# YuhuaXu/ImageMosaicing

Measured on AMD Instinct MI355X. Metric: image-pairs/sec (detect+match+H+warp), 4000x3000 UAV frames, higher is better.
Workload: dtype i16 fixed-point pyramid filtered in f32 (as the reference's OpenCV), f32 (RANSAC / warp coordinates), int8 MFMA with int32 accumulation (descriptor distances, exact), u8 (pixels); 1 GPU; C3: ONE 500-frame 4000x3000 UAV survey, pair window 2 (499 pairs), SIFT(2000,3,0.01,20) + exact BF match + 3x3 grid select + Ransac2D + MosaicImagesRefined warp; frames=500, pairs=499, frames_per_gpu=500, pairs_per_gpu=499

## Files before the change

imagemosaicing_amd/csrc/sift.hip:

```cpp
#include "common.h"
#include <memory>
#include "detmath.h"
#include <cmath>
#include <type_traits>

namespace {

constexpr int N_LAYERS = 3, N_LEVELS = 6, IMG_BORDER = 5, MAX_INTERP = 5, ORI_BINS = 36, MAX_OCT = 16;
constexpr int FIXPT_SCALE = 48;
constexpr float DOG_THRESHOLD_P1 = 21.0f;
constexpr float HIST_Q = 1024.0f;
constexpr int MAX_R = 16;
constexpr int SIFT_BATCH_MAX = MI355_SIFT_BATCH_MAX;
typedef int16_t lvl_t;

__host__ __device__ __forceinline__ int reflect101(int p, int n) {
    if (n == 1) return 0;
    while (p < 0 || p >= n) { if (p < 0) p = -p; else p = 2 * n - 2 - p; }
    return p;
}

typedef float v2f __attribute__((ext_vector_type(2)));
struct __attribute__((aligned(4))) uint2_a4 { unsigned x, y; };
typedef float v4f __attribute__((ext_vector_type(4)));

__device__ __forceinline__ v4f ld4(const lvl_t* p) {
    const uint2 q = *reinterpret_cast<const uint2*>(p);
    v4f o;
    o.x = (float)(int)(short)(q.x & 0xffffu); o.y = (float)((int)q.x >> 16);
    o.z = (float)(int)(short)(q.y & 0xffffu); o.w = (float)((int)q.y >> 16);
    return o;
}
__device__ __forceinline__ float ld1(const lvl_t* p) { return (float)(int)*p; }
__device__ __forceinline__ int sat16(float v) {
    int q = (int)rintf(v);
    q = q < -32768 ? -32768 : (q > 32767 ? 32767 : q);
    return q;
}
__device__ __forceinline__ float gray48(const uint8_t* p) {
    return (float)(((1868 * (int)p[0] + 9617 * (int)p[1] + 4899 * (int)p[2] + 8192) >> 14) * FIXPT_SCALE);
}

__device__ __forceinline__ int xcd_remap(int bid, int nb) {
    const int q = nb >> 3, r = nb & 7, xcd = bid & 7, local = bid >> 3;
    const int base = xcd < r ? xcd * (q + 1) : r * (q + 1) + (xcd - r) * q;
    return base + local;
}

template <int J, int NPP, class F> __device__ __forceinline__ bool static_rows(F& f) {
    if constexpr (J < NPP) { if (!f(std::integral_constant<int, J>{})) return false; return static_rows<J + 1, NPP>(f); }
    else return true;
}

struct Blur16Args {
    const lvl_t* src;
    const uint8_t* bgr[SIFT_BATCH_MAX];
    int bgr_ws[SIFT_BATCH_MAX];
    lvl_t* dst;
    lvl_t* ds;
    int w, h;
    int tiles_x, tiles_y;
    float k[2 * MAX_R + 1];
    float kp[2 * (MAX_R + 1)];
    size_t fstride;
    int nb;
};

constexpr int T16W = 64, T16H = 32;
template <int R, bool BGR>
__global__ __launch_bounds__(256) void blur16_tile(Blur16Args a) {
    constexpr int ROWS = T16H + 2 * R, COLS = T16W + 2 * R, PIN = COLS | 1, PMID = T16W + 4;
    __shared__ float s_in[ROWS * PIN];
    __shared__ __attribute__((aligned(16))) float s_mid[ROWS * PMID];
    const int tid = threadIdx.x, fr = blockIdx.y;
    const int tile = xcd_remap(blockIdx.x, a.tiles_x * a.tiles_y);
    const int ty = tile / a.tiles_x, tx = tile - ty * a.tiles_x;
    const int x0 = tx * T16W, y0 = ty * T16H;
    const lvl_t* src = BGR ? nullptr : a.src + (size_t)fr * a.fstride;
    const uint8_t* bgr = a.bgr[0]; int bws = a.bgr_ws[0];
    if (BGR) {
#pragma unroll
        for (int q = 1; q < SIFT_BATCH_MAX; q++) if (fr == q) { bgr = a.bgr[q]; bws = a.bgr_ws[q]; }
    }
    lvl_t* dst = a.dst + (size_t)fr * a.fstride;
    for (int idx = tid; idx < ROWS * COLS; idx += 256) {
        const int ry = idx / COLS, rx = idx - ry * COLS;
        const int gy = reflect101(y0 - R + ry, a.h), gx = reflect101(x0 - R + rx, a.w);
        s_in[ry * PIN + rx] = BGR ? gray48(bgr + (size_t)gy * bws + 3 * gx) : ld1(src + (size_t)gy * a.w + gx);
    }
    __syncthreads();
    for (int item = tid; item < ROWS * (T16W / 4); item += 256) {
        const int xg = item / ROWS, row = item - xg * ROWS;
        const float* in = s_in + row * PIN + 4 * xg;
        float e[2 * R + 4];
#pragma unroll
        for (int m = 0; m < 2 * R + 4; m++) e[m] = in[m];
        float acc[4];
#pragma unroll
        for (int q = 0; q < 4; q++) acc[q] = a.k[0] * e[q];
#pragma unroll
        for (int i = 1; i <= 2 * R; i++) {
#pragma unroll
            for (int q = 0; q < 4; q++) { const float p = a.k[i] * e[q + i]; acc[q] = acc[q] + p; }
        }
        *reinterpret_cast<v4f*>(s_mid + row * PMID + 4 * xg) = (v4f){acc[0], acc[1], acc[2], acc[3]};
    }
    __syncthreads();
    for (int item = tid; item < T16H * (T16W / 4); item += 256) {
        const int yy = item / (T16W / 4), xg = item - yy * (T16W / 4);
        const float* mid = s_mid + (yy + R) * PMID + 4 * xg;
        v4f acc = *reinterpret_cast<const v4f*>(mid) * a.k[R];
#pragma unroll
        for (int j = 1; j <= R; j++) {
            const v4f sm = *reinterpret_cast<const v4f*>(mid + j * PMID) + *reinterpret_cast<const v4f*>(mid - j * PMID);
            const v4f p = sm * a.k[R + j];
            acc = acc + p;
        }
        const int gx = x0 + 4 * xg, gy = y0 + yy;
        if (gy >= a.h) continue;
        const int o0 = sat16(acc.x), o1 = sat16(acc.y), o2 = sat16(acc.z), o3 = sat16(acc.w);
        lvl_t* d = dst + (size_t)gy * a.w + gx;
        if (gx + 3 < a.w && (a.w & 3) == 0) {
            *reinterpret_cast<uint2*>(d) = make_uint2((unsigned)(o0 & 0xffff) | ((unsigned)o1 << 16), (unsigned)(o2 & 0xffff) | ((unsigned)o3 << 16));
        } else {
            if (gx < a.w) d[0] = (lvl_t)o0;
            if (gx + 1 < a.w) d[1] = (lvl_t)o1;
            if (gx + 2 < a.w) d[2] = (lvl_t)o2;
            if (gx + 3 < a.w) d[3] = (lvl_t)o3;
        }
        if (a.ds && !(gy & 1) && (gy >> 1) < (a.h >> 1)) {
            lvl_t* q = a.ds + (size_t)fr * a.fstride + (size_t)(gy >> 1) * (a.w >> 1);
            if ((gx >> 1) < (a.w >> 1)) q[gx >> 1] = (lvl_t)o0;
            if (((gx + 2) >> 1) < (a.w >> 1)) q[(gx + 2) >> 1] = (lvl_t)o2;
        }
    }
}

#include "build/blur16_asm.inc"
template <int R, bool BGR, bool DS>
__device__ __forceinline__ void blur16_stream_body(const Blur16Args& a, int L, int nstrip, int nseg) {
    constexpr int RA = (R + 3) / 4 * 4, SW = 256, BW = SW + 2 * RA;
    constexpr int BUF = (BW + 8 + 63) & ~63;
    static_assert(2 * RA + R <= 64, "halo lanes");
    __shared__ __attribute__((aligned(16))) float s_buf[4][2][BUF];
    const int lane = threadIdx.x & 63, wave = threadIdx.x >> 6;
    int unit = __builtin_amdgcn_readfirstlane(xcd_remap(blockIdx.x, gridDim.x) * 4 + wave);
    const int per = nstrip * nseg, fr = unit / per;
    if (fr >= a.nb) return;
    unit -= fr * per;
    const int seg = unit / nstrip, strip = unit - seg * nstrip;
    if (seg >= nseg) return;
    const int x0 = strip * SW, y0 = seg * L;
    const int lact = (a.h - y0 < L) ? a.h - y0 : L;
    const int wv = a.w - x0;
    const int xm = x0 + 4 * lane;
    const int xl = xm < a.w - 4 ? xm : a.w - 4;
    int hcol, hpos;
    if (lane < RA) { hcol = x0 - RA + lane; hpos = lane; }
    else if (lane < 2 * RA) { hcol = x0 + SW + (lane - RA); hpos = SW + lane; }
    else if (wv < SW && lane < 2 * RA + R) { hcol = x0 + wv + (lane - 2 * RA); hpos = RA + wv + (lane - 2 * RA); }
    else { hcol = x0; hpos = BW + (lane & 7); }
    hcol = reflect101(hcol, a.w);
    const size_t fro = (size_t)fr * a.fstride;
    const uint8_t* bgr = a.bgr[0]; int bws = a.bgr_ws[0];
    if (BGR) {
#pragma unroll
        for (int q = 1; q < SIFT_BATCH_MAX; q++) if (fr == q) { bgr = a.bgr[q]; bws = a.bgr_ws[q]; }
    }
    const int rowb = BGR ? bws : 2 * a.w;
    int gy = y0 - R, dir = 1;
    if (gy < 0) { gy = -gy; dir = -1; }
    const unsigned long long rp = (unsigned long long)(BGR ? reinterpret_cast<uintptr_t>(bgr) : reinterpret_cast<uintptr_t>(a.src + fro)) + (unsigned long long)gy * (unsigned)rowb;
    const unsigned moff = BGR ? 3u * xl : 2u * xl;
    unsigned hoff, hsh = 0;
    if (BGR) {
        const int b0 = 3 * hcol; int st = b0 & ~3; if (st + 8 > bws) st = bws - 8;
        hoff = (unsigned)st; hsh = 8u * (unsigned)(b0 - st);
    } else hoff = 2u * hcol;
    const unsigned lds0 = (unsigned)reinterpret_cast<uintptr_t>(&s_buf[wave][0][0]);
    const unsigned lds_win = lds0 + 16u * lane, lds_main = lds0 + 4u * (RA + 4 * lane), lds_halo = lds0 + 4u * hpos;
    const unsigned long long dp = (unsigned long long)reinterpret_cast<uintptr_t>(a.dst + fro) + 2ull * (unsigned long long)y0 * a.w;
    const unsigned long long dsp = DS ? (unsigned long long)reinterpret_cast<uintptr_t>(a.ds + fro) + 2ull * (unsigned long long)(y0 >> 1) * (a.w >> 1) : 0ull;
    const unsigned doff = 2u * xm, dsoff = 2u * (xm >> 1);
    const unsigned long long smask = __ballot(xm < a.w);
    const unsigned long long kp = (unsigned long long)reinterpret_cast<uintptr_t>(__builtin_amdgcn_kernarg_segment_ptr()) + offsetof(Blur16Args, kp);
    const int n = lact + 2 * R + 1;
    const int hm1 = a.h - 1, dstr = 2 * a.w;
    (void)hsh;
#define BLUR_ASM_CALL(NAME) NAME(lds_win, lds_main, lds_halo, moff, hoff, doff, dsoff, rp, dp, dsp, kp, smask, rowb, gy, dir, hm1, dstr, n)
    if constexpr (BGR) { static_assert(R == 6, "base level"); blur16_asm_r6_bgr(lds_win, lds_main, lds_halo, moff, hoff, doff, dsoff, hsh, rp, dp, dsp, kp, smask, rowb, gy, dir, hm1, dstr, n); }
    else if constexpr (R == 5) BLUR_ASM_CALL(blur16_asm_r5);
    else if constexpr (R == 6) BLUR_ASM_CALL(blur16_asm_r6);
    else if constexpr (R == 8 && DS) BLUR_ASM_CALL(blur16_asm_r8_ds);
    else if constexpr (R == 8) BLUR_ASM_CALL(blur16_asm_r8);
    else if constexpr (R == 10) BLUR_ASM_CALL(blur16_asm_r10);
    else if constexpr (R == 13) BLUR_ASM_CALL(blur16_asm_r13);
#undef BLUR_ASM_CALL
}
template <int R, bool BGR, bool DS, int W>
__global__ __launch_bounds__(256) __attribute__((amdgpu_waves_per_eu(W, W))) void blur16_stream(Blur16Args a, int L, int nstrip, int nseg) {
    blur16_stream_body<R, BGR, DS>(a, L, nstrip, nseg);
}

__global__ __launch_bounds__(256) void downsample16(const lvl_t* src, int sw, lvl_t* dst, int dw, int dh, size_t fstride) {
    src += (size_t)blockIdx.z * fstride; dst += (size_t)blockIdx.z * fstride;
    const int x = blockIdx.x * 64 + (threadIdx.x & 63), y = blockIdx.y * 4 + (threadIdx.x >> 6);
    if (x < dw && y < dh) dst[(size_t)y * dw + x] = src[(size_t)(2 * y) * sw + 2 * x];
}

struct OctaveDev { lvl_t* lv[N_LEVELS]; int w, h; };

#ifndef EXT_EH
#define EXT_EH 16
#endif
constexpr int EW = 64, EH = EXT_EH, ECAP = 128;
#ifndef REG_SHIFT_V
#define REG_SHIFT_V 0
#endif
constexpr int REG_SHIFT = REG_SHIFT_V;
constexpr int NREG = 64, REG_STRIDE = 32;
struct BatchStride { size_t pyr, claimed, cand, refined, kps, cube, sel, mins; };
constexpr size_t CNT_STRIDE = 64, CCNT_STRIDE = (size_t)64 * 32, SEL_STRIDE = 2048;
struct FrameOuts { mi355_keypoint* kp[SIFT_BATCH_MAX]; uint8_t* d8[SIFT_BATCH_MAX]; };

struct Refined { int o, layer, r, c; float xi, xr, xc, contr, scl; unsigned start; };

struct PyrDev { OctaveDev oc[MAX_OCT]; unsigned* claimed[MAX_OCT]; unsigned* mins[MAX_OCT]; int n_oct; };

__device__ __forceinline__ float dogv(const OctaveDev& oc, size_t foff, int lvl, int r, int c) {
    const size_t o = foff + (size_t)r * oc.w + c;
    return (float)((int)oc.lv[lvl + 1][o] - (int)oc.lv[lvl][o]);
}

__device__ __forceinline__ void solve3(const float a[3][3], const float b[3], float x[3]) {
    const float det = (a[0][0] * (a[1][1] * a[2][2] - a[2][1] * a[1][2]) - a[0][1] * (a[1][0] * a[2][2] - a[2][0] * a[1][2])) + a[0][2] * (a[1][0] * a[2][1] - a[2][0] * a[1][1]);
    if (det == 0.0f) { x[0] = x[1] = x[2] = 0.0f; return; }
    const float d = 1.0f / det;
    x[0] = d * ((b[0] * (a[1][1] * a[2][2] - a[1][2] * a[2][1]) - a[0][1] * (b[1] * a[2][2] - a[1][2] * b[2])) + a[0][2] * (b[1] * a[2][1] - a[1][1] * b[2]));
    x[1] = d * ((a[0][0] * (b[1] * a[2][2] - a[1][2] * b[2]) - b[0] * (a[1][0] * a[2][2] - a[1][2] * a[2][0])) + a[0][2] * (a[1][0] * b[2] - b[1] * a[2][0]));
    x[2] = d * ((a[0][0] * (a[1][1] * b[2] - b[1] * a[2][1]) - a[0][1] * (a[1][0] * b[2] - b[1] * a[2][0])) + b[0] * (a[1][0] * a[2][1] - a[1][1] * a[2][0]));
}

struct FitOff { float xi, xr, xc; };
template <class DV>
__device__ __forceinline__ FitOff fit_step(DV dv, int L, int R, int C) {
    const float img_scale = 1.0f / (float)(255 * FIXPT_SCALE);
    const float deriv_scale = img_scale * 0.5f, second_scale = img_scale, cross_scale = img_scale * 0.25f;
    float dD[3];
    dD[0] = (dv(L, R, C + 1) - dv(L, R, C - 1)) * deriv_scale;
    dD[1] = (dv(L, R + 1, C) - dv(L, R - 1, C)) * deriv_scale;
    dD[2] = (dv(L + 1, R, C) - dv(L - 1, R, C)) * deriv_scale;
    const float v2 = dv(L, R, C) * 2.0f;
    const float dxx = (dv(L, R, C + 1) + dv(L, R, C - 1) - v2) * second_scale;
    const float dyy = (dv(L, R + 1, C) + dv(L, R - 1, C) - v2) * second_scale;
// ... 220 lines not shown
#pragma unroll
    for (int b = 0; b < 12; b++) out |= ((hit >> (11 - b)) & 1u) << b;
    unsigned cmask = 0;
#pragma unroll
    for (int k = 0; k < 4; k++) cmask |= (xm + k >= clo && xm + k < chi) ? (0x111u << k) : 0u;
    return out & cmask;
}

struct XH { s2 hx[5][2], hn[5][2]; };
struct XCen { s2 v[3][2]; };
__device__ __forceinline__ void xrow_extremes(const XDog& d, XH& h, XCen& c) {
#pragma unroll
    for (int p = 0; p < 5; p++) {
        const unsigned u01 = as_u(d.m[p][0]), u23 = as_u(d.m[p][1]);
        const unsigned l23 = dpp_lower(u23), r01 = dpp_upper(u01);
        const s2 s_m0 = as_s2(__builtin_amdgcn_alignbit(u01, l23, 16));
        const s2 s_12 = as_s2(__builtin_amdgcn_alignbit(u23, u01, 16));
        const s2 s_34 = as_s2(__builtin_amdgcn_alignbit(r01, u23, 16));
        h.hx[p][0] = pmax(pmax(s_m0, d.m[p][0]), s_12); h.hx[p][1] = pmax(pmax(s_12, d.m[p][1]), s_34);
        h.hn[p][0] = pmin(pmin(s_m0, d.m[p][0]), s_12); h.hn[p][1] = pmin(pmin(s_12, d.m[p][1]), s_34);
    }
#pragma unroll
    for (int l = 0; l < 3; l++) { c.v[l][0] = d.m[l + 1][0]; c.v[l][1] = d.m[l + 1][1]; }
}
__device__ __forceinline__ unsigned xtest_rows(const XH& A, const XH& B, const XH& C, const XCen& cen, int xm, int clo, int chi, bool row_ok) {
    s2 hx[5][2], hn[5][2];
#pragma unroll
    for (int p = 0; p < 5; p++)
#pragma unroll
        for (int r = 0; r < 2; r++) { hx[p][r] = pmax(pmax(A.hx[p][r], B.hx[p][r]), C.hx[p][r]); hn[p][r] = pmin(pmin(A.hn[p][r], B.hn[p][r]), C.hn[p][r]); }
    unsigned hit = 0;
    const s2 t21 = {21, 21}, tm21 = {-21, -21};
#pragma unroll
    for (int layer = 1; layer <= N_LAYERS; layer++) {
#pragma unroll
        for (int r = 0; r < 2; r++) {
            const s2 val = cen.v[layer - 1][r];
            const s2 mx = pmax(pmax(pmax(hx[layer - 1][r], hx[layer][r]), hx[layer + 1][r]), t21);
            const s2 mn = pmin(pmin(pmin(hn[layer - 1][r], hn[layer][r]), hn[layer + 1][r]), tm21);
            const bool h0 = (val.x == mx.x) | (val.x == mn.x), h1 = (val.y == mx.y) | (val.y == mn.y);
            hit = (hit << 2) | (h0 ? 2u : 0u) | (h1 ? 1u : 0u);
        }
    }
    if (!row_ok || hit == 0) return 0u;
    unsigned out = 0;
#pragma unroll
    for (int b = 0; b < 12; b++) out |= ((hit >> (11 - b)) & 1u) << b;
    unsigned cmask = 0;
#pragma unroll
    for (int k = 0; k < 4; k++) cmask |= (xm + k >= clo && xm + k < chi) ? (0x111u << k) : 0u;
    return out & cmask;
}

__global__ __launch_bounds__(256) __attribute__((amdgpu_waves_per_eu(XWAVES, XWAVES)))
void extrema_stream(OctaveDev oc, int octave, unsigned long long* cand, unsigned* count, unsigned cap, unsigned* overflow, BatchStride bs,
                    float* cube, unsigned cube_cap, int L, int nstrip, int nseg, int nb, int xsw ) {
    const int lane = threadIdx.x & 63, wave = threadIdx.x >> 6;
    int unit = __builtin_amdgcn_readfirstlane(xcd_remap(blockIdx.x, gridDim.x) * 4 + wave);
    const int per = nstrip * nseg, fr = unit / per;
    if (fr >= nb) return;
    unit -= fr * per;
    {
        const size_t f = (size_t)fr;
#pragma unroll
        for (int l = 0; l < N_LEVELS; l++) oc.lv[l] += f * bs.pyr;
        cand += f * bs.cand; count += f * CCNT_STRIDE; overflow += f * CNT_STRIDE; cube += f * bs.cube;
    }
    const int seg = unit / nstrip, strip = unit - seg * nstrip;
    const int xs = strip * xsw, y0 = seg * L;
    const int lact = (oc.h - y0 < L) ? oc.h - y0 : L;
    const unsigned reg = (unsigned)unit & (NREG - 1);
    const int xm = xs - 4 + 4 * lane;
    const int xl = xm < 0 ? 0 : (xm < oc.w - 4 ? xm : oc.w - 4);
    int clo = xs > IMG_BORDER ? xs : IMG_BORDER, chi = xs + xsw < oc.w - IMG_BORDER ? xs + xsw : oc.w - IMG_BORDER;
    if (lane == 0 || lane == 63) { clo = 0; chi = 0; }
    const int hm1 = oc.h - 1;
    auto load_row = [&](int r, XRow& q) {
        r = r < 0 ? 0 : (r > hm1 ? hm1 : r);
        const size_t o = (size_t)r * oc.w + xl;
#pragma unroll
        for (int l = 0; l < N_LEVELS; l++) q.m[l] = *reinterpret_cast<const uint2*>(oc.lv[l] + o);
    };
    auto to_dog = [&](const XRow& q, XDog& d) {
#pragma unroll
        for (int p = 0; p < 5; p++) { d.m[p][0] = as_s2(q.m[p + 1].x) - as_s2(q.m[p].x); d.m[p][1] = as_s2(q.m[p + 1].y) - as_s2(q.m[p].y); }
    };
    __shared__ unsigned long long s_rec[4][XCAP];
    int nq = 0;
    auto wave_sync = [&]() { __builtin_amdgcn_fence(__ATOMIC_ACQ_REL, "wavefront"); __builtin_amdgcn_wave_barrier(); };
    auto flush = [&]() {
        if (nq == 0) return;
        wave_sync();
        unsigned base = 0;
        if (lane == 0) base = atomicAdd(&count[reg * REG_STRIDE], (unsigned)nq);
        base = __shfl(base, 0);
        for (int idx = lane; idx < nq; idx += 64) {
            const unsigned g = base + (unsigned)idx;
            if (g >= cap) { *overflow = 1; continue; }
            cand[(size_t)reg * cap + g] = s_rec[wave][idx];
        }
        wave_sync();
        nq = 0;
    };
    auto emit = [&](unsigned hit, int rc, auto in_loop) -> bool {
        constexpr bool IN_LOOP = decltype(in_loop)::value;
        const int nq0 = nq;
        while (__builtin_amdgcn_ballot_w64(hit != 0)) {
            const bool mine = hit != 0;
            const int bb = mine ? __builtin_ctz(hit) : 0;
            hit &= hit - 1;
            const unsigned long long m = __builtin_amdgcn_ballot_w64(mine);
// ... 750 lines not shown
        if (q < 2) v = v + (float)(long long)s_hq[idx + n + q] * (1.0f / HIST_Q);
        s_dst[t] = v;
    }
    wave_sync();
    float a = s_dst[lane], b = s_dst[lane + 64];
    auto seq_sum = [&](float va, float vb) {
        const float sa = va * va, sb = vb * vb;
        float acc = 0.0f;
#pragma unroll
        for (int q = 0; q < 64; q++) acc = acc + __int_as_float(__builtin_amdgcn_readlane(__float_as_int(sa), q));
#pragma unroll
        for (int q = 0; q < 64; q++) acc = acc + __int_as_float(__builtin_amdgcn_readlane(__float_as_int(sb), q));
        return acc;
    };
    const float thr = sqrtf(seq_sum(a, b)) * 0.2f;
    a = a < thr ? a : thr; b = b < thr ? b : thr;
    const float nn = sqrtf(seq_sum(a, b));
    const float fac = 512.0f / (nn > 1.1920929e-7f ? nn : 1.1920929e-7f);
    const float va = rintf(a * fac), vb = rintf(b * fac);
    desc[(size_t)kidx * 128 + lane] = (uint8_t)(va < 0.0f ? 0 : (va > 255.0f ? 255 : (int)va));
    desc[(size_t)kidx * 128 + lane + 64] = (uint8_t)(vb < 0.0f ? 0 : (vb > 255.0f ? 255 : (int)vb));
}

int gauss_kernel_host(double sigma, float* k) {
    const int ksize = ((int)lrint(sigma * 8.0 + 1.0)) | 1;
    const int r = ksize / 2;
    double sum = 0.0;
    const double scale2x = -0.5 / (sigma * sigma);
    for (int i = 0; i < ksize; i++) { const double x = (double)i - (double)(ksize - 1) * 0.5; k[i] = (float)std::exp(scale2x * x * x); sum += (double)k[i]; }
    sum = 1.0 / sum;
    for (int i = 0; i < ksize; i++) k[i] = (float)((double)k[i] * sum);
    return r;
}

inline bool blur_streams(const Blur16Args& a, bool bgr, int R, int stream_mode) {
    const bool has_r = bgr ? R == 6 : (R == 5 || R == 6 || R == 8 || R == 10 || R == 13);
    bool ok = stream_mode && has_r && (a.w & 3) == 0 && ((a.w & 255) == 0 || (a.w & 255) > MAX_R) && a.w >= 512 && a.h >= 64;
    if (bgr) { for (int f = 0; f < a.nb; f++) ok = ok && ((uintptr_t)a.bgr[f] & 3) == 0 && (a.bgr_ws[f] & 3) == 0 && a.bgr_ws[f] >= 3 * a.w; }
    else ok = ok && ((uintptr_t)a.src & 7) == 0;
    if (a.ds) ok = ok && R == 8 && (a.h & 1) == 0;
    return ok && ((uintptr_t)a.dst & 7) == 0 && (a.fstride & 3) == 0;
}
inline void stream_grid(int w, int h, int& L, int& nstrip, int& nseg, int nb = 1, int waves = 2) {
    static const int units_env = [] { const char* e = getenv("MI355_STREAM_UNITS"); return e ? atoi(e) : 0; }();
    const int units_target = units_env ? units_env : 1024 * waves;
    static const int stream_minl = [] { const char* e = getenv("MI355_STREAM_MINL"); return e ? atoi(e) : 64; }();
    nstrip = (w + 255) / 256;
    nseg = (units_target + nstrip * nb - 1) / (nstrip * nb);
    L = (h + nseg - 1) / nseg;
    if (L < stream_minl) L = stream_minl;
    L = (L + 1) & ~1;
    nseg = (h + L - 1) / L;
}
template <bool BGR>
bool launch_blur(hipStream_t st, int R, const Blur16Args& a_in, int stream_mode, bool* streamed = nullptr) {
    Blur16Args a = a_in;
    const int nb = a.nb > 1 ? a.nb : 1;
    if (streamed) *streamed = false;
    if (blur_streams(a, BGR, R, stream_mode)) {
        static const int w4 = [] { const char* e = getenv("MI355_STREAM_W4"); return e ? atoi(e) : 8; }();
        const int waves = (R <= w4 && R <= 8) ? 4 : 3;
        double ksum = 0.0;
        for (int t = 0; t <= 2 * R; t++) ksum += std::fabs((double)a.k[t]);
        if (ksum < 2.6) {
            for (int t = 0; t <= R; t++) { a.kp[2 * t] = a.k[t]; a.kp[2 * t + 1] = t ? a.k[t - 1] : 0.0f; }
            int L, nstrip, nseg;
            stream_grid(a.w, a.h, L, nstrip, nseg, nb, waves);
            const int units = nstrip * nseg * nb;
            const dim3 grid((units + 3) / 4), block(256);
            if (streamed) *streamed = true;
#define LAUNCH(RR, DS, WW) hipLaunchKernelGGL((blur16_stream<RR, BGR, DS, WW>), grid, block, 0, st, a, L, nstrip, nseg); return true
            if constexpr (BGR) { if (waves == 4) { LAUNCH(6, false, 4); } else { LAUNCH(6, false, 3); } }
            else {
                switch (R) {
                    case 5: if (waves == 4) { LAUNCH(5, false, 4); } else { LAUNCH(5, false, 3); }
                    case 6: if (waves == 4) { LAUNCH(6, false, 4); } else { LAUNCH(6, false, 3); }
                    case 8: if (a.ds) { if (waves == 4) { LAUNCH(8, true, 4); } else { LAUNCH(8, true, 3); } }
                            else { if (waves == 4) { LAUNCH(8, false, 4); } else { LAUNCH(8, false, 3); } }
                    case 10: LAUNCH(10, false, 3);
                    case 13: LAUNCH(13, false, 3);
                    default: break;
                }
            }
#undef LAUNCH
        }
    }
    const dim3 grid(a.tiles_x * a.tiles_y, nb), block(256);
    switch (R) {
#define CASE(RR) case RR: hipLaunchKernelGGL((blur16_tile<RR, BGR>), grid, block, 0, st, a); return true;
        CASE(2) CASE(3) CASE(4) CASE(5) CASE(6) CASE(7) CASE(8) CASE(9) CASE(10) CASE(11) CASE(12) CASE(13) CASE(14) CASE(15) CASE(16)
#undef CASE
        default: return false;
    }
}

}

struct SiftWork {
    int w = 0, h = 0;
    int nb = 0;
    int n_oct = 0;
    hipStream_t stream = nullptr;
    hipEvent_t done = nullptr;
    DevBuf pyr;
    DevBuf claimed;
    DevBuf cand, refined, kps, kresp, sel, counters, rhist, ccnt;
    DevBuf olist;
    DevBuf mins; bool keepall = false;
    int kmax = 0;
    DevBuf ksort; size_t ksort_stride = 0;
    DevBuf cube; unsigned cube_cap = 0;
    PyrDev P;
    BatchStride bs;
    unsigned cand_cap = 0, ref_cap = 0, kp_cap = 0;
    float kern[N_LEVELS][2 * MAX_R + 1];
    int radius[N_LEVELS];
    float kern0[2 * MAX_R + 1]; int radius0 = 0;
    struct Pend { int img_id; const uint8_t* d_bgr; int ws; hipEvent_t ev; };
    std::vector<Pend> pend;
};

constexpr int SIFT_SLOTS_MAX = 4;
#define SIFT_SLOTS (ctx->sift_nslots)

void mi_sift_release(mi355_ctx* ctx) {
    for (SiftWork* s : ctx->sift_slots) {
        if (!s) continue;
        if (s->stream) { (void)hipStreamSynchronize(s->stream); (void)hipStreamDestroy(s->stream); }
        if (s->done) (void)hipEventDestroy(s->done);
        s->pyr.release(); s->claimed.release(); s->cand.release(); s->refined.release(); s->kps.release(); s->kresp.release(); s->sel.release(); s->counters.release(); s->rhist.release(); s->ccnt.release(); s->cube.release(); s->olist.release(); s->mins.release(); s->ksort.release();
        delete s;
    }
    ctx->sift_slots.clear();
    if (ctx->sift_in_ev) { (void)hipEventDestroy(ctx->sift_in_ev); ctx->sift_in_ev = nullptr; }
    for (int* p : ctx->pinned_chunks) (void)hipHostFree(p);
    ctx->pinned_chunks.clear();
    ctx->pinned_used = 0;
}
// ... 189 lines not shown
    f.w = w; f.h = h;
    MI_HIP(f.kp.reserve(sizeof(mi355_keypoint) * (size_t)(keepall ? kmax : 2048)));
    MI_HIP(f.d8.reserve((size_t)128 * (size_t)(keepall ? kmax : 2048)));
    f.pending = true; f.h_cnt = nullptr; f.ready = nullptr; f.n = 0;
    s->pend.push_back({img_id, d_bgr, ws, ctx->pend_event});
    if ((int)s->pend.size() >= nb) {
        rc = sift_run_batch(ctx, s);
        if (rc != MI355_OK) return rc;
    }
    if (ctx->pinned_used >= PINNED_CHUNK * 64) {
        rc = mi_resolve_features(ctx);
        if (rc != MI355_OK) return rc;
        ctx->pinned_used = 0;
    }
    if (n_kp) {
        rc = mi_resolve_features(ctx);
        if (rc != MI355_OK) return rc;
        *n_kp = f.n;
    }
    return MI355_OK;
}

static int sift_run_batch(mi355_ctx* ctx, SiftWork* s) {
    std::vector<SiftWork::Pend> pend;
    pend.swap(s->pend);
    const int n = (int)pend.size();
    if (n == 0) return MI355_OK;
    ctx->sift_next = (ctx->sift_next + 1) % SIFT_SLOTS;
    const hipStream_t st = s->stream;
    const hipStream_t tt = st;
    const int w = s->w, h = s->h;
    const int nf = ctx->p.nfeatures;
    const BatchStride bs = s->bs;
    MI_HIP(hipEventRecord(ctx->sift_in_ev, ctx->stream));
    MI_HIP(hipStreamWaitEvent(st, ctx->sift_in_ev, 0));
    const bool serial_heavy = ctx->serial_heavy != 0;
    if (serial_heavy && ctx->heavy_ev_valid) MI_HIP(hipStreamWaitEvent(st, ctx->heavy_ev, 0));
    unsigned* cnt = s->counters.as<unsigned>();
    MI_HIP(hipMemsetAsync(cnt, 0, (size_t)n * CNT_STRIDE * sizeof(unsigned), st));
    MI_HIP(hipMemsetAsync(s->ccnt.p, 0, (size_t)n * CCNT_STRIDE * sizeof(unsigned), st));
    FrameOuts outs;
    memset(&outs, 0, sizeof(outs));
    std::vector<Features*> fs(n);
    for (int k = 0; k < n; k++) {
        fs[k] = &ctx->feats[pend[k].img_id];
        outs.kp[k] = fs[k]->kp.as<mi355_keypoint>(); outs.d8[k] = fs[k]->d8.as<uint8_t>();
    }
    auto blur_args = [&](const OctaveDev& oc) {
        Blur16Args a; memset(&a, 0, sizeof(a));
        a.w = oc.w; a.h = oc.h; a.tiles_x = (oc.w + T16W - 1) / T16W; a.tiles_y = (oc.h + T16H - 1) / T16H;
        a.fstride = bs.pyr; a.nb = n;
        return a;
    };
    bool ds_fused = false;
    for (int o = 0; o < s->n_oct; o++) {
        const OctaveDev& oc = s->P.oc[o];
        const double level_bytes = (double)oc.w * oc.h * sizeof(lvl_t) * n;
        if (o == 0) {
            Blur16Args a = blur_args(oc);
            for (int k = 0; k < n; k++) { a.bgr[k] = pend[k].d_bgr; a.bgr_ws[k] = pend[k].ws; }
            a.dst = oc.lv[0];
            memcpy(a.k, s->kern0, sizeof(float) * (2 * s->radius0 + 1));
            const bool streams = blur_streams(a, true, s->radius0, ctx->blur_stream);
            ProfScope ps(ctx, streams ? "gauss_stream" : "gauss", level_bytes + (double)w * h * 3.0 * n, st);
            if (!launch_blur<true>(st, s->radius0, a, ctx->blur_stream)) { ctx->set_error("sift: unsupported kernel radius"); return MI355_ERR_FAILED; }
        } else if (!ds_fused) {
            const OctaveDev& pv = s->P.oc[o - 1];
            ProfScope ps(ctx, "downsample", level_bytes * 2.0, st);
            hipLaunchKernelGGL(downsample16, dim3((oc.w + 63) / 64, (oc.h + 3) / 4, n), dim3(256), 0, st, pv.lv[N_LAYERS], pv.w, oc.lv[0], oc.w, oc.h, bs.pyr);
        }
        ds_fused = false;
        for (int i = 1; i < N_LEVELS; i++) {
            Blur16Args a = blur_args(oc);
            a.src = oc.lv[i - 1]; a.dst = oc.lv[i];
            memcpy(a.k, s->kern[i], sizeof(float) * (2 * s->radius[i] + 1));
            if (i == N_LAYERS && o + 1 < s->n_oct && (oc.w & 3) == 0 && (s->P.oc[o + 1].w == (oc.w >> 1)) && (s->P.oc[o + 1].h == (oc.h >> 1))) {
                a.ds = s->P.oc[o + 1].lv[0]; ds_fused = true;
                if (!blur_streams(a, false, s->radius[i], ctx->blur_stream)) {
                    Blur16Args b = a; b.ds = nullptr;
                    if (blur_streams(b, false, s->radius[i], ctx->blur_stream)) { a.ds = nullptr; ds_fused = false; }
                }
            }
            const bool streams = blur_streams(a, false, s->radius[i], ctx->blur_stream);
            ProfScope ps(ctx, streams ? "gauss_stream" : "gauss", level_bytes * 2.0, st);
            if (!launch_blur<false>(st, s->radius[i], a, ctx->blur_stream)) { ctx->set_error("sift: unsupported kernel radius"); return MI355_ERR_FAILED; }
        }
        {
            ProfScope ps(ctx, "extrema", level_bytes * 6.0, st);
            const bool xs = ctx->blur_stream && (oc.w & 3) == 0 && oc.w >= ctx->xstream_min_w && oc.h >= ctx->xstream_min_w * 3 / 4 && n >= ctx->xstream_min_frames;
            if (xs) {
                const int nstrip = (oc.w + XSW - 1) / XSW;
                const int xsw = ((oc.w + nstrip - 1) / nstrip + 3) & ~3;
                int nseg = 1, L = oc.h;
                for (int k = 2; k >= 1; k--) {
                    const int ns = (1024 * XWAVES * k) / (nstrip * n);
                    if (ns < 1) continue;
                    const int l = (oc.h + ns - 1) / ns;
                    if (l >= 64 || k == 1) { L = l < 64 ? 64 : l; break; }
                }
                nseg = (oc.h + L - 1) / L;
                hipLaunchKernelGGL(extrema_stream, dim3((nstrip * nseg * n + 3) / 4), dim3(256), 0, st,
                                   oc, o, s->cand.as<unsigned long long>(), s->ccnt.as<unsigned>(), s->cand_cap, cnt + 4, bs, s->cube.as<float>(), s->cube_cap, L, nstrip, nseg, n, xsw);
            } else {
                hipLaunchKernelGGL(extrema_kernel, dim3(((oc.w + EW - 1) / EW) * ((oc.h + EH - 1) / EH), n), dim3(256), 0, st,
                                   oc, o, s->cand.as<unsigned long long>(), s->ccnt.as<unsigned>(), s->cand_cap, cnt + 4, bs, s->cube.as<float>(), s->cube_cap);
            }
        }
    }
    if (serial_heavy) {
        if (!ctx->heavy_ev) MI_HIP(hipEventCreateWithFlags(&ctx->heavy_ev, hipEventDisableTiming));
        MI_HIP(hipEventRecord(ctx->heavy_ev, st)); ctx->heavy_ev_valid = true;
    }
    {
        ProfScope ps(ctx, "refine", 0.0, tt);
        static const int refine_gx = [] { const char* e = getenv("MI355_REFINE_GX"); return e ? atoi(e) : 2; }();
        hipLaunchKernelGGL(refine_kernel, dim3(refine_gx, NREG, n), dim3(256), 0, tt, s->P, s->cand.as<unsigned long long>(), s->ccnt.as<unsigned>(), s->cand_cap, cnt + 0,
                           ctx->p.contrast_threshold, ctx->p.edge_threshold, 1.6f, s->refined.as<Refined>(), cnt + 1, s->ref_cap, s->rhist.as<unsigned>(), bs, s->cube.as<float>(), s->cube_cap);
    }
    if (s->keepall) {
        {
            ProfScope ps(ctx, "kp_select", 0.0, tt);
            hipLaunchKernelGGL(keepall_live_kernel, dim3(256, n), dim3(256), 0, tt, s->P, s->refined.as<Refined>(), cnt + 1, s->ref_cap, cnt + 8, s->olist.as<unsigned>(), bs);
            hipLaunchKernelGGL(keepall_reset_kernel, dim3(256, n), dim3(256), 0, tt, s->P, s->refined.as<Refined>(), cnt + 1, s->ref_cap, bs);
        }
        {
            ProfScope ps(ctx, "orient", 0.0, tt);
            hipLaunchKernelGGL(orient_kernel, dim3(ctx->num_cu * 4, n), dim3(256), 0, tt, s->P, s->refined.as<Refined>(), cnt + 1, s->ref_cap,
                               s->kps.as<KpRec>(), s->kresp.as<unsigned>(), cnt + 2, s->kp_cap, cnt + 8, 0, bs, s->olist.as<unsigned>());
        }
        {
            ProfScope ps(ctx, "topk", 0.0, tt);
            const unsigned kmax = (unsigned)s->kmax;
            if (ctx->keepall_order == 1) {
                hipLaunchKernelGGL(keepall_output_kernel, dim3((kmax + 255) / 256, n), dim3(256), 0, tt, s->kps.as<KpRec>(), cnt + 2, s->kp_cap, kmax, outs, s->sel.as<SelRec>(),
                                   reinterpret_cast<int*>(cnt + 3), reinterpret_cast<int*>(cnt + 4), bs);
            } else {
                hipLaunchKernelGGL(keepall_sort_tiles_kernel, dim3((kmax + KA_TILE - 1) / KA_TILE, n), dim3(1024), 0, tt, s->kps.as<KpRec>(), cnt + 2, s->kp_cap, kmax,
                                   s->ksort.as<unsigned long long>(), s->ksort_stride, outs, s->sel.as<SelRec>(), bs);
                hipLaunchKernelGGL(keepall_place_kernel, dim3((kmax + 255) / 256, n), dim3(256), 0, tt, s->kps.as<KpRec>(), cnt + 2, s->kp_cap, kmax,
                                   s->ksort.as<const unsigned long long>(), s->ksort_stride, outs, s->sel.as<SelRec>(), reinterpret_cast<int*>(cnt + 3), reinterpret_cast<int*>(cnt + 4), bs);
            }
        }
    } else {
    {
        ProfScope ps(ctx, "kp_select", 0.0, tt);
        hipLaunchKernelGGL(select_unclaim_kernel, dim3(1 + UNCLAIM_WGS, n), dim3(1024), 0, tt, s->P, s->refined.as<Refined>(), bs, s->rhist.as<unsigned>(), cnt + 1, s->ref_cap, (unsigned)nf + 256u, cnt + 8,
                           bs.refined, s->olist.as<unsigned>());
    }
    for (int pass = 0; pass < 2; pass++) {
        {
            ProfScope ps(ctx, "orient", 0.0, tt);
            hipLaunchKernelGGL(orient_kernel, dim3(ctx->num_cu * 4, n), dim3(256), 0, tt, s->P, s->refined.as<Refined>(), cnt + 1, s->ref_cap,
                               s->kps.as<KpRec>(), s->kresp.as<unsigned>(), cnt + 2, s->kp_cap, cnt + 8, pass, bs, s->olist.as<unsigned>());
        }
        {
            ProfScope ps(ctx, "topk", 0.0, tt);
            hipLaunchKernelGGL(topk_kernel, dim3(n), dim3(1024), 0, tt, s->kps.as<KpRec>(), s->kresp.as<unsigned>(), cnt + 2, s->kp_cap, nf,
                               outs, s->sel.as<SelRec>(), reinterpret_cast<int*>(cnt + 3), reinterpret_cast<int*>(cnt + 4), cnt + 8, pass, bs);
        }
    }
// ... 44 lines not shown
```

Before: 3904 image-pairs/s.

## Merge blur levels 4-5 and extrema across first three octaves into shared launches

Reorders the pyramid build so the first few octaves are seeded and blurred up to level 3. The level-4 and level-5 Gaussian blurs, and the extrema search, for those octaves are then each issued as one multi-part streaming launch. A part table in kernel arguments maps block ranges to octaves, and each part's L is rebalanced to fill the device. This cuts launch count and tail underutilisation on the smaller octaves. In exchange it adds per-block part selection overhead and a larger kernarg, and it changes launch order, so smaller octaves now also use the stream extrema kernel (min width lowered to 512).

```diff
diff --git a/imagemosaicing_amd/csrc/sift.hip b/imagemosaicing_amd/csrc/sift.hip
--- a/imagemosaicing_amd/csrc/sift.hip
+++ b/imagemosaicing_amd/csrc/sift.hip
@@ -52,6 +52,15 @@
     else return true;
 }
 
+constexpr int STREAM_PARTS_MAX = 3;
+struct StreamPart {
+    const lvl_t* src; lvl_t* dst;
+    size_t fstride;
+    int w, h;
+    int nstrip, nseg, L;
+    int unit0;
+};
+struct StreamParts { StreamPart p[STREAM_PARTS_MAX]; int n; };
 struct Blur16Args {
     const lvl_t* src;
     const uint8_t* bgr[SIFT_BATCH_MAX];
@@ -64,7 +73,22 @@
     float kp[2 * (MAX_R + 1)];
     size_t fstride;
     int nb;
+    StreamParts t;
 };
+#define STREAM_PART_SEL(T, PI, F) ((PI) == 0 ? (T).p[0].F : ((PI) == 1 ? (T).p[1].F : (T).p[2].F))
+__device__ __forceinline__ int uniform(int v) { return __builtin_amdgcn_readfirstlane(v); }
+__device__ __forceinline__ size_t uniform(size_t v) {
+    return ((size_t)(unsigned)__builtin_amdgcn_readfirstlane((int)(v >> 32)) << 32) | (size_t)(unsigned)__builtin_amdgcn_readfirstlane((int)v);
+}
+template <class P> __device__ __forceinline__ P* uniform(P* v) { return reinterpret_cast<P*>(uniform((size_t)reinterpret_cast<uintptr_t>(v))); }
+template <class Table>
+__device__ __forceinline__ int stream_part_of(const Table& t, int bid, int nblocks, int& b0, int& nblk) {
+    const int b1 = t.n > 1 ? t.p[1].unit0 >> 2 : nblocks, b2 = t.n > 2 ? t.p[2].unit0 >> 2 : nblocks;
+    const int pi = (bid >= b1 ? 1 : 0) + (bid >= b2 ? 1 : 0);
+    b0 = pi == 0 ? 0 : (pi == 1 ? b1 : b2);
+    nblk = uniform((pi == 0 ? b1 : (pi == 1 ? b2 : nblocks)) - b0); b0 = uniform(b0);
+    return uniform(pi);
+}
 
 constexpr int T16W = 64, T16H = 32;
 template <int R, bool BGR>
@@ -138,39 +162,48 @@
 
 #include "build/blur16_asm.inc"
 template <int R, bool BGR, bool DS>
-__device__ __forceinline__ void blur16_stream_body(const Blur16Args& a, int L, int nstrip, int nseg) {
+__device__ __forceinline__ void blur16_stream_body(const Blur16Args& a) {
     constexpr int RA = (R + 3) / 4 * 4, SW = 256, BW = SW + 2 * RA;
     constexpr int BUF = (BW + 8 + 63) & ~63;
     static_assert(2 * RA + R <= 64, "halo lanes");
     __shared__ __attribute__((aligned(16))) float s_buf[4][2][BUF];
     const int lane = threadIdx.x & 63, wave = threadIdx.x >> 6;
-    int unit = __builtin_amdgcn_readfirstlane(xcd_remap(blockIdx.x, gridDim.x) * 4 + wave);
+    typedef const __attribute__((address_space(4))) StreamParts* parts_ptr;
+    const parts_ptr tp = (parts_ptr)((const __attribute__((address_space(4))) char*)__builtin_amdgcn_kernarg_segment_ptr() + offsetof(Blur16Args, t));
+    int pb0, nblk;
+    const int pi = stream_part_of(*tp, (int)blockIdx.x, (int)gridDim.x, pb0, nblk);
+    const int w = uniform(tp->p[pi].w), h = uniform(tp->p[pi].h), L = uniform(tp->p[pi].L);
+    const int nstrip = uniform(tp->p[pi].nstrip), nseg = uniform(tp->p[pi].nseg);
+    const lvl_t* const psrc = uniform(tp->p[pi].src);
+    lvl_t* const pdst = uniform(tp->p[pi].dst);
+    const size_t fstride = uniform(tp->p[pi].fstride);
+    int unit = __builtin_amdgcn_readfirstlane(xcd_remap((int)blockIdx.x - pb0, nblk) * 4 + wave);
     const int per = nstrip * nseg, fr = unit / per;
     if (fr >= a.nb) return;
     unit -= fr * per;
     const int seg = unit / nstrip, strip = unit - seg * nstrip;
     if (seg >= nseg) return;
     const int x0 = strip * SW, y0 = seg * L;
-    const int lact = (a.h - y0 < L) ? a.h - y0 : L;
-    const int wv = a.w - x0;
+    const int lact = (h - y0 < L) ? h - y0 : L;
+    const int wv = w - x0;
     const int xm = x0 + 4 * lane;
-    const int xl = xm < a.w - 4 ? xm : a.w - 4;
+    const int xl = xm < w - 4 ? xm : w - 4;
     int hcol, hpos;
     if (lane < RA) { hcol = x0 - RA + lane; hpos = lane; }
     else if (lane < 2 * RA) { hcol = x0 + SW + (lane - RA); hpos = SW + lane; }
     else if (wv < SW && lane < 2 * RA + R) { hcol = x0 + wv + (lane - 2 * RA); hpos = RA + wv + (lane - 2 * RA); }
     else { hcol = x0; hpos = BW + (lane & 7); }
-    hcol = reflect101(hcol, a.w);
-    const size_t fro = (size_t)fr * a.fstride;
+    hcol = reflect101(hcol, w);
+    const size_t fro = (size_t)fr * fstride;
     const uint8_t* bgr = a.bgr[0]; int bws = a.bgr_ws[0];
     if (BGR) {
 #pragma unroll
         for (int q = 1; q < SIFT_BATCH_MAX; q++) if (fr == q) { bgr = a.bgr[q]; bws = a.bgr_ws[q]; }
     }
-    const int rowb = BGR ? bws : 2 * a.w;
+    const int rowb = BGR ? bws : 2 * w;
     int gy = y0 - R, dir = 1;
     if (gy < 0) { gy = -gy; dir = -1; }
-    const unsigned long long rp = (unsigned long long)(BGR ? reinterpret_cast<uintptr_t>(bgr) : reinterpret_cast<uintptr_t>(a.src + fro)) + (unsigned long long)gy * (unsigned)rowb;
+    const unsigned long long rp = (unsigned long long)(BGR ? reinterpret_cast<uintptr_t>(bgr) : reinterpret_cast<uintptr_t>(psrc + fro)) + (unsigned long long)gy * (unsigned)rowb;
     const unsigned moff = BGR ? 3u * xl : 2u * xl;
     unsigned hoff, hsh = 0;
     if (BGR) {
@@ -179,13 +212,13 @@
     } else hoff = 2u * hcol;
     const unsigned lds0 = (unsigned)reinterpret_cast<uintptr_t>(&s_buf[wave][0][0]);
     const unsigned lds_win = lds0 + 16u * lane, lds_main = lds0 + 4u * (RA + 4 * lane), lds_halo = lds0 + 4u * hpos;
-    const unsigned long long dp = (unsigned long long)reinterpret_cast<uintptr_t>(a.dst + fro) + 2ull * (unsigned long long)y0 * a.w;
-    const unsigned long long dsp = DS ? (unsigned long long)reinterpret_cast<uintptr_t>(a.ds + fro) + 2ull * (unsigned long long)(y0 >> 1) * (a.w >> 1) : 0ull;
+    const unsigned long long dp = (unsigned long long)reinterpret_cast<uintptr_t>(pdst + fro) + 2ull * (unsigned long long)y0 * w;
+    const unsigned long long dsp = DS ? (unsigned long long)reinterpret_cast<uintptr_t>(a.ds + fro) + 2ull * (unsigned long long)(y0 >> 1) * (w >> 1) : 0ull;
     const unsigned doff = 2u * xm, dsoff = 2u * (xm >> 1);
-    const unsigned long long smask = __ballot(xm < a.w);
+    const unsigned long long smask = __ballot(xm < w);
     const unsigned long long kp = (unsigned long long)reinterpret_cast<uintptr_t>(__builtin_amdgcn_kernarg_segment_ptr()) + offsetof(Blur16Args, kp);
     const int n = lact + 2 * R + 1;
-    const int hm1 = a.h - 1, dstr = 2 * a.w;
+    const int hm1 = h - 1, dstr = 2 * w;
     (void)hsh;
 #define BLUR_ASM_CALL(NAME) NAME(lds_win, lds_main, lds_halo, moff, hoff, doff, dsoff, rp, dp, dsp, kp, smask, rowb, gy, dir, hm1, dstr, n)
     if constexpr (BGR) { static_assert(R == 6, "base level"); blur16_asm_r6_bgr(lds_win, lds_main, lds_halo, moff, hoff, doff, dsoff, hsh, rp, dp, dsp, kp, smask, rowb, gy, dir, hm1, dstr, n); }
@@ -198,8 +231,8 @@
 #undef BLUR_ASM_CALL
 }
 template <int R, bool BGR, bool DS, int W>
-__global__ __launch_bounds__(256) __attribute__((amdgpu_waves_per_eu(W, W))) void blur16_stream(Blur16Args a, int L, int nstrip, int nseg) {
-    blur16_stream_body<R, BGR, DS>(a, L, nstrip, nseg);
+__global__ __launch_bounds__(256) __attribute__((amdgpu_waves_per_eu(W, W))) void blur16_stream(Blur16Args a) {
+    blur16_stream_body<R, BGR, DS>(a);
 }
 
 __global__ __launch_bounds__(256) void downsample16(const lvl_t* src, int sw, lvl_t* dst, int dw, int dh, size_t fstride) {
@@ -526,11 +559,25 @@
     return out & cmask;
 }
 
+struct XStreamPart {
+    OctaveDev oc; int octave;
+    int nstrip, nseg, L, xsw;
+    int unit0;
+};
+struct XStreamParts { XStreamPart p[STREAM_PARTS_MAX]; int n; };
 __global__ __launch_bounds__(256) __attribute__((amdgpu_waves_per_eu(XWAVES, XWAVES)))
-void extrema_stream(OctaveDev oc, int octave, unsigned long long* cand, unsigned* count, unsigned cap, unsigned* overflow, BatchStride bs,
-                    float* cube, unsigned cube_cap, int L, int nstrip, int nseg, int nb, int xsw ) {
+void extrema_stream(XStreamParts t, unsigned long long* cand, unsigned* count, unsigned cap, unsigned* overflow, BatchStride bs,
+                    float* cube, unsigned cube_cap, int nb) {
     const int lane = threadIdx.x & 63, wave = threadIdx.x >> 6;
-    int unit = __builtin_amdgcn_readfirstlane(xcd_remap(blockIdx.x, gridDim.x) * 4 + wave);
+    int pb0, nblk;
+    const int pi = stream_part_of(t, (int)blockIdx.x, (int)gridDim.x, pb0, nblk);
+    OctaveDev oc;
+#pragma unroll
+    for (int l = 0; l < N_LEVELS; l++) oc.lv[l] = STREAM_PART_SEL(t, pi, oc.lv[l]);
+    oc.w = STREAM_PART_SEL(t, pi, oc.w); oc.h = STREAM_PART_SEL(t, pi, oc.h);
+    const int octave = STREAM_PART_SEL(t, pi, octave), L = STREAM_PART_SEL(t, pi, L), xsw = STREAM_PART_SEL(t, pi, xsw);
+    const int nstrip = STREAM_PART_SEL(t, pi, nstrip), nseg = STREAM_PART_SEL(t, pi, nseg);
+    int unit = __builtin_amdgcn_readfirstlane(xcd_remap((int)blockIdx.x - pb0, nblk) * 4 + wave);
     const int per = nstrip * nseg, fr = unit / per;
     if (fr >= nb) return;
     unit -= fr * per;
@@ -1387,38 +1434,78 @@
     L = (L + 1) & ~1;
     nseg = (h + L - 1) / L;
 }
+inline bool stream_taps_ok(const Blur16Args& a, int R) {
+    double ksum = 0.0;
+    for (int t = 0; t <= 2 * R; t++) ksum += std::fabs((double)a.k[t]);
+    return ksum < 2.6;
+}
+inline int stream_waves(int R) {
+    static const int w4 = [] { const char* e = getenv("MI355_STREAM_W4"); return e ? atoi(e) : 8; }();
+    return (R <= w4 && R <= 8) ? 4 : 3;
+}
+inline int stream_merge_mode() {
+    static const int v = [] { const char* e = getenv("MI355_STREAM_MERGE"); return e ? atoi(e) : 1; }();
+    return v;
+}
+template <bool BGR>
+void launch_blur_stream(hipStream_t st, int R, const Blur16Args* parts, int np) {
+    Blur16Args a = parts[0];
+    const int nb = a.nb > 1 ? a.nb : 1, waves = stream_waves(R);
+    for (int t = 0; t <= R; t++) { a.kp[2 * t] = a.k[t]; a.kp[2 * t + 1] = t ? a.k[t - 1] : 0.0f; }
+    StreamParts& tb = a.t;
+    int units = 0;
+    for (int p = 0; p < np; p++) {
+        StreamPart& q = tb.p[p];
+        q.src = parts[p].src; q.dst = parts[p].dst; q.fstride = parts[p].fstride; q.w = parts[p].w; q.h = parts[p].h;
+        stream_grid(q.w, q.h, q.L, q.nstrip, q.nseg, nb, waves);
+    }
+    if (np > 1) {
+        for (int L = 64; ; L += 2) {
+            int u = 0;
+            for (int p = 0; p < np; p++) u += tb.p[p].nstrip * ((tb.p[p].h + L - 1) / L) * nb;
+            if (u <= 1024 * waves || L >= tb.p[0].h) {
+                for (int p = 0; p < np; p++) {
+                    StreamPart& q = tb.p[p];
+                    q.nseg = (q.h + L - 1) / L;
+                    q.L = ((q.h + q.nseg - 1) / q.nseg + 1) & ~1;
+                    if (q.L < 64) q.L = 64;
+                    q.nseg = (q.h + q.L - 1) / q.L;
+                }
+                break;
+            }
+        }
+    }
+    for (int p = 0; p < np; p++) {
+        StreamPart& q = tb.p[p];
+        q.unit0 = p ? (units + 31) & ~31 : 0;
+        units = q.unit0 + q.nstrip * q.nseg * nb;
+    }
+    tb.n = np;
+    const dim3 grid((units + 3) / 4), block(256);
+#define LAUNCH(RR, DS, WW) hipLaunchKernelGGL((blur16_stream<RR, BGR, DS, WW>), grid, block, 0, st, a); return
+    if constexpr (BGR) { if (waves == 4) { LAUNCH(6, false, 4); } else { LAUNCH(6, false, 3); } }
+    else {
+        switch (R) {
+            case 5: if (waves == 4) { LAUNCH(5, false, 4); } else { LAUNCH(5, false, 3); }
+            case 6: if (waves == 4) { LAUNCH(6, false, 4); } else { LAUNCH(6, false, 3); }
+            case 8: if (a.ds) { if (waves == 4) { LAUNCH(8, true, 4); } else { LAUNCH(8, true, 3); } }
+                    else { if (waves == 4) { LAUNCH(8, false, 4); } else { LAUNCH(8, false, 3); } }
+            case 10: LAUNCH(10, false, 3);
+            case 13: LAUNCH(13, false, 3);
+            default: break;
+        }
+    }
+#undef LAUNCH
+}
 template <bool BGR>
 bool launch_blur(hipStream_t st, int R, const Blur16Args& a_in, int stream_mode, bool* streamed = nullptr) {
     Blur16Args a = a_in;
     const int nb = a.nb > 1 ? a.nb : 1;
     if (streamed) *streamed = false;
-    if (blur_streams(a, BGR, R, stream_mode)) {
-        static const int w4 = [] { const char* e = getenv("MI355_STREAM_W4"); return e ? atoi(e) : 8; }();
-        const int waves = (R <= w4 && R <= 8) ? 4 : 3;
-        double ksum = 0.0;
-        for (int t = 0; t <= 2 * R; t++) ksum += std::fabs((double)a.k[t]);
-        if (ksum < 2.6) {
-            for (int t = 0; t <= R; t++) { a.kp[2 * t] = a.k[t]; a.kp[2 * t + 1] = t ? a.k[t - 1] : 0.0f; }
-            int L, nstrip, nseg;
-            stream_grid(a.w, a.h, L, nstrip, nseg, nb, waves);
-            const int units = nstrip * nseg * nb;
-            const dim3 grid((units + 3) / 4), block(256);
-            if (streamed) *streamed = true;
-#define LAUNCH(RR, DS, WW) hipLaunchKernelGGL((blur16_stream<RR, BGR, DS, WW>), grid, block, 0, st, a, L, nstrip, nseg); return true
-            if constexpr (BGR) { if (waves == 4) { LAUNCH(6, false, 4); } else { LAUNCH(6, false, 3); } }
-            else {
-                switch (R) {
-                    case 5: if (waves == 4) { LAUNCH(5, false, 4); } else { LAUNCH(5, false, 3); }
-                    case 6: if (waves == 4) { LAUNCH(6, false, 4); } else { LAUNCH(6, false, 3); }
-                    case 8: if (a.ds) { if (waves == 4) { LAUNCH(8, true, 4); } else { LAUNCH(8, true, 3); } }
-                            else { if (waves == 4) { LAUNCH(8, false, 4); } else { LAUNCH(8, false, 3); } }
-                    case 10: LAUNCH(10, false, 3);
-                    case 13: LAUNCH(13, false, 3);
-                    default: break;
-                }
-            }
-#undef LAUNCH
-        }
+    if (blur_streams(a, BGR, R, stream_mode) && stream_taps_ok(a, R)) {
+        if (streamed) *streamed = true;
+        launch_blur_stream<BGR>(st, R, &a, 1);
+        return true;
     }
     const dim3 grid(a.tiles_x * a.tiles_y, nb), block(256);
     switch (R) {
@@ -1714,10 +1801,12 @@
         a.fstride = bs.pyr; a.nb = n;
         return a;
     };
+    const char* radius_err = "sift: unsupported kernel radius";
     bool ds_fused = false;
-    for (int o = 0; o < s->n_oct; o++) {
+    auto seed_level = [&](int o) -> bool {
         const OctaveDev& oc = s->P.oc[o];
         const double level_bytes = (double)oc.w * oc.h * sizeof(lvl_t) * n;
+        bool ok = true;
         if (o == 0) {
             Blur16Args a = blur_args(oc);
             for (int k = 0; k < n; k++) { a.bgr[k] = pend[k].d_bgr; a.bgr_ws[k] = pend[k].ws; }
@@ -1725,49 +1814,116 @@
             memcpy(a.k, s->kern0, sizeof(float) * (2 * s->radius0 + 1));
             const bool streams = blur_streams(a, true, s->radius0, ctx->blur_stream);
             ProfScope ps(ctx, streams ? "gauss_stream" : "gauss", level_bytes + (double)w * h * 3.0 * n, st);
-            if (!launch_blur<true>(st, s->radius0, a, ctx->blur_stream)) { ctx->set_error("sift: unsupported kernel radius"); return MI355_ERR_FAILED; }
+            ok = launch_blur<true>(st, s->radius0, a, ctx->blur_stream);
         } else if (!ds_fused) {
             const OctaveDev& pv = s->P.oc[o - 1];
             ProfScope ps(ctx, "downsample", level_bytes * 2.0, st);
             hipLaunchKernelGGL(downsample16, dim3((oc.w + 63) / 64, (oc.h + 3) / 4, n), dim3(256), 0, st, pv.lv[N_LAYERS], pv.w, oc.lv[0], oc.w, oc.h, bs.pyr);
         }
         ds_fused = false;
-        for (int i = 1; i < N_LEVELS; i++) {
-            Blur16Args a = blur_args(oc);
-            a.src = oc.lv[i - 1]; a.dst = oc.lv[i];
-            memcpy(a.k, s->kern[i], sizeof(float) * (2 * s->radius[i] + 1));
-            if (i == N_LAYERS && o + 1 < s->n_oct && (oc.w & 3) == 0 && (s->P.oc[o + 1].w == (oc.w >> 1)) && (s->P.oc[o + 1].h == (oc.h >> 1))) {
-                a.ds = s->P.oc[o + 1].lv[0]; ds_fused = true;
-                if (!blur_streams(a, false, s->radius[i], ctx->blur_stream)) {
-                    Blur16Args b = a; b.ds = nullptr;
-                    if (blur_streams(b, false, s->radius[i], ctx->blur_stream)) { a.ds = nullptr; ds_fused = false; }
-                }
-            }
-            const bool streams = blur_streams(a, false, s->radius[i], ctx->blur_stream);
-            ProfScope ps(ctx, streams ? "gauss_stream" : "gauss", level_bytes * 2.0, st);
-            if (!launch_blur<false>(st, s->radius[i], a, ctx->blur_stream)) { ctx->set_error("sift: unsupported kernel radius"); return MI355_ERR_FAILED; }
-        }
-        {
-            ProfScope ps(ctx, "extrema", level_bytes * 6.0, st);
-            const bool xs = ctx->blur_stream && (oc.w & 3) == 0 && oc.w >= ctx->xstream_min_w && oc.h >= ctx->xstream_min_w * 3 / 4 && n >= ctx->xstream_min_frames;
-            if (xs) {
-                const int nstrip = (oc.w + XSW - 1) / XSW;
-                const int xsw = ((oc.w + nstrip - 1) / nstrip + 3) & ~3;
-                int nseg = 1, L = oc.h;
-                for (int k = 2; k >= 1; k--) {
-                    const int ns = (1024 * XWAVES * k) / (nstrip * n);
-                    if (ns < 1) continue;
-                    const int l = (oc.h + ns - 1) / ns;
-                    if (l >= 64 || k == 1) { L = l < 64 ? 64 : l; break; }
-                }
-                nseg = (oc.h + L - 1) / L;
-                hipLaunchKernelGGL(extrema_stream, dim3((nstrip * nseg * n + 3) / 4), dim3(256), 0, st,
-                                   oc, o, s->cand.as<unsigned long long>(), s->ccnt.as<unsigned>(), s->cand_cap, cnt + 4, bs, s->cube.as<float>(), s->cube_cap, L, nstrip, nseg, n, xsw);
-            } else {
-                hipLaunchKernelGGL(extrema_kernel, dim3(((oc.w + EW - 1) / EW) * ((oc.h + EH - 1) / EH), n), dim3(256), 0, st,
-                                   oc, o, s->cand.as<unsigned long long>(), s->ccnt.as<unsigned>(), s->cand_cap, cnt + 4, bs, s->cube.as<float>(), s->cube_cap);
-            }
-        }
+        return ok;
+    };
+    auto level_args = [&](int o, int i) {
+        const OctaveDev& oc = s->P.oc[o];
+        Blur16Args a = blur_args(oc);
+        a.src = oc.lv[i - 1]; a.dst = oc.lv[i];
+        memcpy(a.k, s->kern[i], sizeof(float) * (2 * s->radius[i] + 1));
+        return a;
+    };
+    auto blur_level = [&](int o, int i) -> bool {
+        const OctaveDev& oc = s->P.oc[o];
+        const double level_bytes = (double)oc.w * oc.h * sizeof(lvl_t) * n;
+        Blur16Args a = level_args(o, i);
+        if (i == N_LAYERS && o + 1 < s->n_oct && (oc.w & 3) == 0 && (s->P.oc[o + 1].w == (oc.w >> 1)) && (s->P.oc[o + 1].h == (oc.h >> 1))) {
+            a.ds = s->P.oc[o + 1].lv[0]; ds_fused = true;
+            if (!blur_streams(a, false, s->radius[i], ctx->blur_stream)) {
+                Blur16Args b = a; b.ds = nullptr;
+                if (blur_streams(b, false, s->radius[i], ctx->blur_stream)) { a.ds = nullptr; ds_fused = false; }
+            }
+        }
+        const bool streams = blur_streams(a, false, s->radius[i], ctx->blur_stream);
+        ProfScope ps(ctx, streams ? "gauss_stream" : "gauss", level_bytes * 2.0, st);
+        return launch_blur<false>(st, s->radius[i], a, ctx->blur_stream);
+    };
+    auto extrema_streams = [&](int o, bool rider) {
+        const OctaveDev& oc = s->P.oc[o];
+        const int min_w = rider && ctx->xstream_min_w > 512 ? 512 : ctx->xstream_min_w;
+        return ctx->blur_stream && (oc.w & 3) == 0 && oc.w >= min_w && oc.h >= min_w * 3 / 4 && n >= ctx->xstream_min_frames;
+    };
+    auto extrema = [&](const int* os, int np, bool streamed) {
+        double bytes = 0.0;
+        for (int p = 0; p < np; p++) bytes += (double)s->P.oc[os[p]].w * s->P.oc[os[p]].h * sizeof(lvl_t) * n * 6.0;
+        ProfScope ps(ctx, "extrema", bytes, st);
+        if (!streamed) {
+            const OctaveDev& oc = s->P.oc[os[0]];
+            hipLaunchKernelGGL(extrema_kernel, dim3(((oc.w + EW - 1) / EW) * ((oc.h + EH - 1) / EH), n), dim3(256), 0, st,
+                               oc, os[0], s->cand.as<unsigned long long>(), s->ccnt.as<unsigned>(), s->cand_cap, cnt + 4, bs, s->cube.as<float>(), s->cube_cap);
+            return;
+        }
+        XStreamParts tb; memset(&tb, 0, sizeof(tb));
+        int units = 0;
+        for (int p = 0; p < np; p++) {
+            XStreamPart& q = tb.p[p];
+            q.oc = s->P.oc[os[p]]; q.octave = os[p];
+            q.nstrip = (q.oc.w + XSW - 1) / XSW;
+            q.xsw = ((q.oc.w + q.nstrip - 1) / q.nstrip + 3) & ~3;
+            q.L = q.oc.h;
+            for (int k = 2; k >= 1; k--) {
+                const int ns = (1024 * XWAVES * k) / (q.nstrip * n);
+                if (ns < 1) continue;
+                const int l = (q.oc.h + ns - 1) / ns;
+                if (l >= 64 || k == 1) { q.L = l < 64 ? 64 : l; break; }
+            }
+            q.nseg = (q.oc.h + q.L - 1) / q.L;
+            q.unit0 = p ? (units + 31) & ~31 : 0;
+            units = q.unit0 + q.nstrip * q.nseg * n;
+        }
+        tb.n = np;
+        hipLaunchKernelGGL(extrema_stream, dim3((units + 3) / 4), dim3(256), 0, st,
+                           tb, s->cand.as<unsigned long long>(), s->ccnt.as<unsigned>(), s->cand_cap, cnt + 4, bs, s->cube.as<float>(), s->cube_cap, n);
+    };
+    const int lv_merge[2] = {N_LAYERS + 1, N_LAYERS + 2};
+    bool part_blur[2][STREAM_PARTS_MAX] = {}, part_x[STREAM_PARTS_MAX] = {};
+    int n_spine = 0;
+    if (stream_merge_mode() && ctx->blur_stream) {
+        int cnt_m[3] = {0, 0, 0}, last = -1;
+        for (int o = 0; o < STREAM_PARTS_MAX && o < s->n_oct; o++) {
+            for (int j = 0; j < 2; j++) {
+                const Blur16Args a = level_args(o, lv_merge[j]);
+                part_blur[j][o] = blur_streams(a, false, s->radius[lv_merge[j]], ctx->blur_stream) && stream_taps_ok(a, s->radius[lv_merge[j]]);
+                cnt_m[j] += part_blur[j][o];
+            }
+            part_x[o] = o == 0 ? extrema_streams(0, false) : (part_x[0] && extrema_streams(o, true));
+            cnt_m[2] += part_x[o];
+            if (part_blur[0][o] || part_blur[1][o] || part_x[o]) last = o;
+        }
+        if (cnt_m[0] > 1 || cnt_m[1] > 1 || cnt_m[2] > 1) n_spine = last + 1;
+    }
+    for (int o = 0; o < n_spine; o++) {
+        if (!seed_level(o)) { ctx->set_error(radius_err); return MI355_ERR_FAILED; }
+        for (int i = 1; i <= N_LAYERS; i++) if (!blur_level(o, i)) { ctx->set_error(radius_err); return MI355_ERR_FAILED; }
+    }
+    if (n_spine) {
+        for (int j = 0; j < 2; j++) {
+            const int i = lv_merge[j];
+            Blur16Args parts[STREAM_PARTS_MAX]; int np = 0;
+            double bytes = 0.0;
+            for (int o = 0; o < n_spine; o++) if (part_blur[j][o]) {
+                parts[np++] = level_args(o, i);
+                bytes += (double)s->P.oc[o].w * s->P.oc[o].h * sizeof(lvl_t) * n * 2.0;
+            }
+            if (np) { ProfScope ps(ctx, "gauss_stream", bytes, st); launch_blur_stream<false>(st, s->radius[i], parts, np); }
+            for (int o = 0; o < n_spine; o++) if (!part_blur[j][o] && !blur_level(o, i)) { ctx->set_error(radius_err); return MI355_ERR_FAILED; }
+        }
+        int os[STREAM_PARTS_MAX], np = 0;
+        for (int o = 0; o < n_spine; o++) if (part_x[o]) os[np++] = o;
+        if (np) extrema(os, np, true);
+        for (int o = 0; o < n_spine; o++) if (!part_x[o]) extrema(&o, 1, false);
+    }
+    for (int o = n_spine; o < s->n_oct; o++) {
+        if (!seed_level(o)) { ctx->set_error(radius_err); return MI355_ERR_FAILED; }
+        for (int i = 1; i < N_LEVELS; i++) if (!blur_level(o, i)) { ctx->set_error(radius_err); return MI355_ERR_FAILED; }
+        extrema(&o, 1, extrema_streams(o, false));
     }
     if (serial_heavy) {
         if (!ctx->heavy_ev) MI_HIP(hipEventCreateWithFlags(&ctx->heavy_ev, hipEventDisableTiming));
```

Result: no change. 3939 image-pairs/s (median of 6 runs) (+0.9%).
